# dmlc/difacto

Hardware: AMD Instinct MI355X
Metric: examples/sec (FM SGD worker step, Criteo-shape, V_dim=64) (higher is better)
Workload: dtype f32

## Files before the change

difacto_amd/csrc/dfh_api.hip:

```cpp
#include <algorithm>
#include <chrono>
#include <cstring>
#include <mutex>
#include <new>
#include <thread>

#include <hip/hip_ext.h>
#include <rocprim/rocprim.hpp>

#include "dfh_kernels.hip"
#include "dfh_localize.hip"
#include "dfh_update.hip"
#include "dfh_riders.hip"

using namespace dfh;

namespace dfh {
static thread_local std::string g_err;
void set_error(const std::string& msg) { g_err = msg; }
}

struct dfh_ctx {
  int device = 0;
  hipStream_t stream = nullptr;
// ... 39 lines not shown

namespace {
struct TimeScope {
  dfh_ctx* c;
  int id;
  hipStream_t st;
  hipEvent_t a = nullptr, b = nullptr;
  static hipEvent_t get(dfh_ctx* c) {
    if (!c->pool.empty()) {
      hipEvent_t e = c->pool.back();
      c->pool.pop_back();
      return e;
    }
    hipEvent_t e = nullptr;
    if (hipEventCreate(&e) != hipSuccess) return nullptr;
    return e;
  }
  TimeScope(dfh_ctx* ctx, int kid, hipStream_t s = nullptr) : c(ctx), id(kid), st(s ? s : ctx->stream) {
    if (kid >= DFH_K_COUNT || !((c->timing >> kid) & 1u)) return;
    a = get(c);
    b = get(c);
    if (a && b) (void)hipEventRecord(a, st);
  }
  ~TimeScope() {
    if (!a || !b) return;
    (void)hipEventRecord(b, st);
    c->spans.push_back({id, a, b});
  }
};
}

struct dfh_table {
  dfh_ctx* ctx = nullptr;
  TableView v{};
  uint64_t hslots = 0;
  uint64_t bytes = 0;
  bool has_aux = true;
  bool auto_grow = false;
  uint64_t rows_bound = 0;
  uint64_t grows = 0;
  uint32_t* d_need = nullptr;
  uint32_t* d_rank = nullptr;
  uint32_t* d_urow = nullptr;
  uint32_t* d_total = nullptr;
  size_t aux_cap = 0;
};

struct dfh_batch {
  dfh_ctx* ctx = nullptr;
  size_t max_rows = 0, max_nnz = 0;
  size_t nrows = 0, nnz = 0;
  bool has_value = false;
  bool has_cnt = false;
  bool localized = false;
  uint64_t* d_raw = nullptr;
  uint32_t* d_offset = nullptr;
  float* d_value = nullptr;
  float* d_label = nullptr;
  void* arena = nullptr;
  void* shared_arena = nullptr;
  size_t arena_bytes = 0;
  uint64_t* o_raw = nullptr;
  uint32_t* o_offset = nullptr;
  float* o_value = nullptr;
  float* o_label = nullptr;
  StageLayout stage;
  char* h_stage = nullptr;
  size_t stage_bytes = 0;
  hipEvent_t ev_staged = nullptr;
  bool staged_pending = false;
  double t_prof[6] = {0, 0, 0, 0, 0, 0};
  uint64_t n_prof = 0;
  char* d_stage_view = nullptr;
  bool defer_ready = false;
  uint64_t *d_keys = nullptr, *d_skeys = nullptr;
  uint32_t *d_pos = nullptr, *d_spos = nullptr;
  uint32_t *d_bpos = nullptr;
  uint32_t *d_head = nullptr, *d_uid = nullptr;
  void* d_temp = nullptr;
  size_t temp_bytes = 0;
  uint64_t *d_smp_key = nullptr, *d_spl_key = nullptr, *d_first_key = nullptr, *d_last_key = nullptr;
  uint32_t *d_smp_rank = nullptr, *d_smp_pos = nullptr, *d_spl_pos = nullptr, *d_packed = nullptr, *d_run_off = nullptr,
           *d_bstart = nullptr, *d_btotal = nullptr, *d_nheads = nullptr, *d_lh = nullptr;
  size_t max_tiles = 0;
  int spl_P = 0;
  uint64_t* d_feaids = nullptr;
  float* d_feacnt = nullptr;
  uint32_t *d_col_ptr = nullptr, *d_index = nullptr, *d_s_row = nullptr;
  float* d_s_val = nullptr;
  uint32_t* d_U = nullptr;
  uint2 *d_mid = nullptr, *d_hot = nullptr, *d_few = nullptr;
  SegEnt *d_mid_ent = nullptr, *d_hot_ent = nullptr, *d_few_ent = nullptr;
  SegEnt* d_split_ent = nullptr;
  uint32_t* d_split_ticket = nullptr;
  float* d_split_part = nullptr;
  size_t split_cap = 0;
  int split_sel = 0, split_last = 0;
  bool split_listing = false;
  uint32_t seg_nb = 0;
  uint2* d_uw = nullptr;
  uint32_t *d_urow = nullptr, *d_need = nullptr, *d_rank = nullptr, *d_total = nullptr;
  float *d_pred = nullptr, *d_slope = nullptr, *d_xv = nullptr;
  size_t xv_floats = 0;
  static constexpr size_t kProgDoubles = 2 * PROG_SLOTS + 64;
  double* d_prog = nullptr;
  float nrows_seen = 0;
  hipEvent_t ev_ready = nullptr, ev_free = nullptr;
  bool ready_pending = false, free_pending = false;
  hipStream_t prep = nullptr;
  bool compute_auc = false;
  uint32_t *d_auc_keys = nullptr, *d_auc_skeys = nullptr, *d_auc_lab = nullptr, *d_auc_slab = nullptr;
  uint32_t* d_auc_part = nullptr;
  uint32_t auc_pending_n = 0;
  bool force_radix = false;
  bool force_sort_fallback = false;
  dfh_table* looked_up = nullptr;
  struct GatherSeg { struct dfh_rowbuf* rb; size_t at, n; };
  std::vector<GatherSeg> gsegs;
  GatherSrc gsrc{};
  bool gather_pending = false, gather_fusable = false, gather_any_value = false, loc_fuse_gather = false;
  const uint32_t *g_rows = nullptr, *g_off = nullptr;
  const float* g_lab = nullptr;
  LocView loc_v{};
  EmitOut loc_o{};
  uint32_t loc_gsort = 0;
  bool loc_big = false;
  int pend_stage = RID_STAGES;
};

namespace dfh {
namespace chunks {
inline hipError_t reset_prog(dfh_batch* b, hipStream_t s);
}
}

namespace {
int flush_pending(dfh_batch* b);
void pend_remove(dfh_ctx* c, dfh_batch* b);
inline hipStream_t prep_of(const dfh_batch* b) {
  const dfh_ctx* c = b->ctx;
  return (c->pipeline && b->prep) ? b->prep : c->stream;
}
void phase_begin(dfh_batch* b) {
  dfh_ctx* c = b->ctx;
  if (b->pend_stage < RID_STAGES) (void)flush_pending(b);
  hipStream_t next = c->pipeline ? c->preps[c->next_prep++ % c->nprep] : nullptr;
  if (next && b->prep && next != b->prep && b->ready_pending) {
    (void)hipStreamWaitEvent(next, b->ev_ready, 0);
  }
  b->prep = next;
}
int prep_begin(dfh_batch* b) {
  dfh_ctx* c = b->ctx;
  if (c->pipeline && !b->prep) phase_begin(b);
  if (c->pipeline && b->free_pending) {
    DFH_HIP(hipStreamWaitEvent(prep_of(b), b->ev_free, 0));
    b->free_pending = false;
  }
  return DFH_OK;
}
int prep_end(dfh_batch* b) {
  dfh_ctx* c = b->ctx;
  if (c->pipeline && !b->defer_ready) {
    DFH_HIP(hipEventRecord(b->ev_ready, prep_of(b)));
    b->ready_pending = true;
  }
// ... 1793 lines not shown
  DFH_ARG(c && (out || size_only) && max_rows >= 1 && max_nnz >= 1, "dfh_batch_create: bad argument");
  DFH_ARG(max_nnz < 0xFFFFFFF0ULL && max_rows < 0xFFFFFFF0ULL, "batch too large for 32-bit positions");
  DFH_HIP(hipSetDevice(c->device));
  dfh_batch* b = new (std::nothrow) dfh_batch();
  DFH_ARG(b != nullptr, "out of host memory");
  b->ctx = c;
  b->max_rows = max_rows;
  b->max_nnz = max_nnz;
  const size_t N = max_nnz, B = max_rows;
  size_t sort_bytes = 0, scan_bytes = 0;
  rocprim::radix_sort_pairs(nullptr, sort_bytes, (uint64_t*)nullptr, (uint64_t*)nullptr, (uint32_t*)nullptr,
                            (uint32_t*)nullptr, N, 0, 64, c->stream);
  rocprim::inclusive_scan(nullptr, scan_bytes, (uint32_t*)nullptr, (uint32_t*)nullptr, N, rocprim::plus<uint32_t>(), c->stream);
  size_t auc_bytes = 0;
  rocprim::radix_sort_pairs(nullptr, auc_bytes, (uint32_t*)nullptr, (uint32_t*)nullptr, (uint32_t*)nullptr,
                            (uint32_t*)nullptr, B, 0, 32, c->stream);
  b->temp_bytes = std::max(std::max(sort_bytes, scan_bytes), auc_bytes) + 256;
  char* arena_at = nullptr;
  size_t arena_need = 0;
  bool sizing = true;
#define DFH_ALLOC(ptr, count, type)                                                        \
  do {                                                                                     \
    const size_t bytes__ = (((size_t)(count) * sizeof(type)) + 255) & ~(size_t)255;        \
    if (sizing) {                                                                          \
      arena_need += bytes__;                                                               \
    } else {                                                                               \
      (ptr) = reinterpret_cast<type*>(arena_at);                                           \
      arena_at += bytes__;                                                                 \
    }                                                                                      \
  } while (0)
  for (int pass = 0; pass < 2; ++pass) {
  sizing = pass == 0;
  if (!sizing) {
    if (size_only) {
      *size_only = arena_need;
      delete b;
      return DFH_OK;
    }
    if (shared) {
      b->shared_arena = shared;
      ++shared->refs;
      arena_at = static_cast<char*>(shared->base) + at;
    } else {
      hipError_t e__ = hipMalloc(reinterpret_cast<void**>(&b->arena), arena_need);
      if (e__ != hipSuccess) {
        set_error(std::string("dfh_batch_create: hipMalloc: ") + hipGetErrorString(e__));
        dfh_batch_destroy(b);
        return DFH_ERR_HIP;
      }
      arena_at = static_cast<char*>(b->arena);
    }
  }
  DFH_ALLOC(b->o_raw, N, uint64_t);
  DFH_ALLOC(b->o_offset, B + 1, uint32_t);
  DFH_ALLOC(b->o_value, N, float);
  DFH_ALLOC(b->o_label, B, float);
  b->d_raw = b->o_raw;
  b->d_offset = b->o_offset;
  b->d_value = b->o_value;
  b->d_label = b->o_label;
  DFH_ALLOC(b->d_keys, N, uint64_t);
  DFH_ALLOC(b->d_skeys, N, uint64_t);
  DFH_ALLOC(b->d_pos, N, uint32_t);
  DFH_ALLOC(b->d_spos, N, uint32_t);
  DFH_ALLOC(b->d_bpos, N, uint32_t);
  DFH_ALLOC(b->d_head, N, uint32_t);
  DFH_ALLOC(b->d_uid, N, uint32_t);
  DFH_ALLOC(b->d_temp, b->temp_bytes, char);
  b->max_tiles = (N + LOC_TILE - 1) / LOC_TILE;
  b->stage = StageLayout(max_rows, max_nnz, b->max_tiles);
  DFH_ALLOC(b->d_spl_key, LOC_BIG_BUCKETS, uint64_t);
  DFH_ALLOC(b->d_spl_pos, LOC_BIG_BUCKETS, uint32_t);
  DFH_ALLOC(b->d_smp_key, LOC_BIG_BUCKETS * LOC_OVERSAMPLE, uint64_t);
  DFH_ALLOC(b->d_smp_pos, LOC_BIG_BUCKETS * LOC_OVERSAMPLE, uint32_t);
  DFH_ALLOC(b->d_smp_rank, LOC_BIG_BUCKETS * LOC_OVERSAMPLE, uint32_t);
  DFH_ALLOC(b->d_first_key, LOC_BIG_BUCKETS, uint64_t);
  DFH_ALLOC(b->d_last_key, LOC_BIG_BUCKETS, uint64_t);
  DFH_ALLOC(b->d_packed, N, uint32_t);
  DFH_ALLOC(b->d_run_off, b->max_tiles * LOC_BIG_BUCKETS, uint32_t);
  DFH_ALLOC(b->d_bstart, LOC_BIG_BUCKETS + 1, uint32_t);
  DFH_ALLOC(b->d_btotal, LOC_XCDS * LOC_BIG_BUCKETS, uint32_t);
  DFH_ALLOC(b->d_nheads, LOC_BIG_BUCKETS, uint32_t);
  DFH_ALLOC(b->d_lh, LOC_BIG_BUCKETS, uint32_t);
  DFH_ALLOC(b->d_feaids, N, uint64_t);
  DFH_ALLOC(b->d_feacnt, N, float);
  DFH_ALLOC(b->d_col_ptr, N + 1, uint32_t);
  DFH_ALLOC(b->d_index, N, uint32_t);
  DFH_ALLOC(b->d_s_row, N, uint32_t);
  DFH_ALLOC(b->d_s_val, N, float);
  DFH_ALLOC(b->d_U, 64, uint32_t);
  DFH_ALLOC(b->d_urow, N, uint32_t);
  DFH_ALLOC(b->d_uw, N, uint2);
  DFH_ALLOC(b->d_mid_ent, N / (BWD_SMALL + 1) + 2 * LOC_BIG_BUCKETS + 16, SegEnt);
  DFH_ALLOC(b->d_hot_ent, N / (BWD_MID + 1) + 2 * LOC_BIG_BUCKETS + 16, SegEnt);
  DFH_ALLOC(b->d_few_ent, N / 2 + 2 * LOC_BIG_BUCKETS + 16, SegEnt);
  b->split_cap = 2 * (N / HOT_SPLIT) + 16;
  DFH_ALLOC(b->d_split_ent, b->split_cap, SegEnt);
  DFH_ALLOC(b->d_split_ticket, b->split_cap, uint32_t);
  DFH_ALLOC(b->d_split_part, b->split_cap * UPD_SPLIT_STRIDE, float);
  DFH_ALLOC(b->d_mid, LOC_BIG_BUCKETS, uint2);
  DFH_ALLOC(b->d_hot, LOC_BIG_BUCKETS, uint2);
  DFH_ALLOC(b->d_few, LOC_BIG_BUCKETS, uint2);
  DFH_ALLOC(b->d_need, N, uint32_t);
  DFH_ALLOC(b->d_rank, N, uint32_t);
  DFH_ALLOC(b->d_pred, B, float);
  DFH_ALLOC(b->d_slope, B, float);
  DFH_ALLOC(b->d_prog, dfh_batch::kProgDoubles, double);
  DFH_ALLOC(b->d_auc_keys, B, uint32_t);
  DFH_ALLOC(b->d_auc_skeys, B, uint32_t);
  DFH_ALLOC(b->d_auc_lab, B, uint32_t);
  DFH_ALLOC(b->d_auc_slab, B, uint32_t);
  DFH_ALLOC(b->d_auc_part, AUC_PART_WORDS, uint32_t);
  }
#undef DFH_ALLOC
  b->arena_bytes = arena_need;
  b->d_total = b->d_U + 1;
  const unsigned evf = hipEventDisableTiming | (c->event_flags ? hipEventDisableSystemFence : 0u);
  hipError_t e2 = hipEventCreateWithFlags(&b->ev_ready, evf);
  if (e2 == hipSuccess) e2 = hipEventCreateWithFlags(&b->ev_free, evf);
  if (e2 == hipSuccess) e2 = chunks::reset_prog(b, c->stream);
  if (e2 == hipSuccess) e2 = hipMemsetAsync(b->d_U, 0, 64 * sizeof(uint32_t), c->stream);
  if (e2 == hipSuccess) e2 = hipMemsetAsync(b->d_split_ticket, 0, b->split_cap * sizeof(uint32_t), c->stream);
  if (e2 == hipSuccess) e2 = hipMemsetAsync(b->d_btotal, 0, LOC_XCDS * LOC_BIG_BUCKETS * sizeof(uint32_t), c->stream);
  if (e2 == hipSuccess) e2 = hipMemsetAsync(b->d_urow, 0xFF, N * sizeof(uint32_t), c->stream);
  if (e2 == hipSuccess) e2 = hipMemsetAsync(b->d_uw, 0xFF, N * sizeof(uint2), c->stream);
  if (e2 == hipSuccess && sync) e2 = hipStreamSynchronize(c->stream);
  if (e2 != hipSuccess) {
    set_error(std::string("dfh_batch_create: ") + hipGetErrorString(e2));
    dfh_batch_destroy(b);
    return DFH_ERR_HIP;
  }
  *out = b;
  return DFH_OK;
}

int dfh_batch_create(dfh_ctx* c, size_t max_rows, size_t max_nnz, dfh_batch** out) {
  return batch_create_impl(c, max_rows, max_nnz, out, nullptr, 0, nullptr, true);
}

int dfh_batch_create_many(dfh_ctx* c, int n, size_t max_rows, size_t max_nnz, dfh_batch** out) {
  DFH_ARG(c && out && n >= 1 && n <= 64, "dfh_batch_create_many: 1 <= n <= 64 objects");
  size_t each = 0;
  int rc = batch_create_impl(c, max_rows, max_nnz, nullptr, nullptr, 0, &each, false);
  if (rc) return rc;
  each = (each + 4095) & ~(size_t)4095;
  SharedArena* sa = new (std::nothrow) SharedArena();
  DFH_ARG(sa != nullptr, "out of host memory");
  DFH_HIP(hipSetDevice(c->device));
  if (hipMalloc(&sa->base, each * (size_t)n) != hipSuccess) {
    delete sa;
    set_error("dfh_batch_create_many: hipMalloc failed");
    return DFH_ERR_HIP;
  }
  for (int i = 0; i < n; ++i) out[i] = nullptr;
  sa->refs = 1;
  for (int i = 0; i < n && !rc; ++i) rc = batch_create_impl(c, max_rows, max_nnz, &out[i], sa, each * (size_t)i, nullptr, false);
  if (!rc && hipStreamSynchronize(c->stream) != hipSuccess) {
    set_error("dfh_batch_create_many: hipStreamSynchronize failed");
    rc = DFH_ERR_HIP;
  }
  if (rc) {
    for (int j = 0; j < n; ++j) {
      if (out[j]) dfh_batch_destroy(out[j]);
      out[j] = nullptr;
    }
  }
// ... 36 lines not shown

extern "C" {

int dfh_batch_load_host(dfh_batch* b, size_t nrows, const size_t* offset, const uint64_t* index, const float* value,
                        const float* label) {
  DFH_ARG(b && offset && label, "dfh_batch_load_host: NULL argument");
  DFH_ARG(nrows >= 1 && nrows <= b->max_rows, "dfh_batch_load_host: nrows out of range");
  std::vector<uint32_t> off32;
  int rc = to_u32_offsets(offset, nrows, &off32);
  if (rc) return rc;
  const size_t base = offset[0], nnz = off32[nrows];
  DFH_ARG(nnz <= b->max_nnz, "dfh_batch_load_host: nnz exceeds max_nnz");
  DFH_ARG(nnz == 0 || index, "index is NULL");
  DFH_HIP(hipSetDevice(b->ctx->device));
  rc = phase_own_arrays(b);
  if (rc) return rc;
  hipStream_t s = prep_of(b);
  const StageLayout& L = b->stage;
  rc = ensure_stage(b, L.load_host_bytes, false);
  if (!rc) rc = stage_wait(b);
  if (rc) return rc;
  memcpy(b->h_stage + L.o_off, off32.data(), (nrows + 1) * 4);
  memcpy(b->h_stage + L.o_lab, label, nrows * 4);
  if (nnz) memcpy(b->h_stage + L.o_idx, index + base, nnz * 8);
  if (nnz && value) memcpy(b->h_stage + L.o_val, value + base, nnz * 4);
  DFH_HIP(hipMemcpyAsync(b->d_offset, b->h_stage + L.o_off, (nrows + 1) * 4, hipMemcpyHostToDevice, s));
  DFH_HIP(hipMemcpyAsync(b->d_label, b->h_stage + L.o_lab, nrows * 4, hipMemcpyHostToDevice, s));
  if (nnz) DFH_HIP(hipMemcpyAsync(b->d_raw, b->h_stage + L.o_idx, nnz * 8, hipMemcpyHostToDevice, s));
  if (nnz && value) DFH_HIP(hipMemcpyAsync(b->d_value, b->h_stage + L.o_val, nnz * 4, hipMemcpyHostToDevice, s));
  DFH_HIP(hipEventRecord(b->ev_staged, s));
  b->staged_pending = true;
  batch_loaded(b, nrows, nnz, value != nullptr);
  return DFH_OK;
}

int dfh_batch_load_device(dfh_batch* b, size_t nrows, size_t nnz, const uint32_t* d_offset, const uint64_t* d_index,
                          const float* d_value, const float* d_label) {
  DFH_ARG(b && d_offset && d_label && (nnz == 0 || d_index), "dfh_batch_load_device: NULL argument");
  DFH_ARG(nrows >= 1 && nrows <= b->max_rows && nnz <= b->max_nnz, "dfh_batch_load_device: shape out of range");
  int rc = phase_own_arrays(b);
  if (rc) return rc;
  hipStream_t s = prep_of(b);
  DFH_HIP(hipMemcpyAsync(b->d_offset, d_offset, (nrows + 1) * 4, hipMemcpyDeviceToDevice, s));
  if (nnz) DFH_HIP(hipMemcpyAsync(b->d_raw, d_index, nnz * 8, hipMemcpyDeviceToDevice, s));
  if (nnz && d_value) DFH_HIP(hipMemcpyAsync(b->d_value, d_value, nnz * 4, hipMemcpyDeviceToDevice, s));
  DFH_HIP(hipMemcpyAsync(b->d_label, d_label, nrows * 4, hipMemcpyDeviceToDevice, s));
  batch_loaded(b, nrows, nnz, d_value != nullptr);
  return DFH_OK;
}

int dfh_batch_attach_device(dfh_batch* b, size_t nrows, size_t nnz, const uint32_t* d_offset, const uint64_t* d_index,
                            const float* d_value, const float* d_label) {
  DFH_ARG(b && d_offset && d_label && (nnz == 0 || d_index), "dfh_batch_attach_device: NULL argument");
  DFH_ARG(nrows >= 1 && nrows <= b->max_rows && nnz <= b->max_nnz, "dfh_batch_attach_device: shape out of range");
  phase_begin(b);
  {
    int rc = prep_begin(b);
    if (rc) return rc;
  }
  b->d_offset = const_cast<uint32_t*>(d_offset);
  b->d_raw = const_cast<uint64_t*>(d_index);
  b->d_value = d_value ? const_cast<float*>(d_value) : b->o_value;
  b->d_label = const_cast<float*>(d_label);
  batch_loaded(b, nrows, nnz, d_value != nullptr);
  return DFH_OK;
}

namespace {
void launch_loc_stage(dfh_batch* b, int stage, hipStream_t s, dfh_table* probe = nullptr) {
  const LocView& v = b->loc_v;
  switch (stage) {
    case RID_COUNT:
      if (b->loc_big) hipLaunchKernelGGL(k_loc_count<LOC_BIG_BUCKETS>, dim3(v.ntiles), dim3(LOC_TILE_THREADS), 0, s, v);
      else if (b->loc_fuse_gather) hipLaunchKernelGGL(k_loc_count_gather<LOC_MAX_BUCKETS>, dim3(v.ntiles), dim3(LOC_TILE_THREADS), 0, s, v, b->gsrc);
      else hipLaunchKernelGGL(k_loc_count<LOC_MAX_BUCKETS>, dim3(v.ntiles), dim3(LOC_TILE_THREADS), 0, s, v);
      break;
    case RID_SCATTER:
      if (b->loc_big) hipLaunchKernelGGL(k_loc_scatter<LOC_BIG_BUCKETS>, dim3(v.ntiles), dim3(LOC_TILE_THREADS), 0, s, v);
      else hipLaunchKernelGGL(k_loc_scatter<LOC_MAX_BUCKETS>, dim3(v.ntiles), dim3(LOC_TILE_THREADS), 0, s, v);
      break;
    case RID_SORT:
      hipLaunchKernelGGL(k_loc_sort, dim3(b->loc_gsort), dim3(LOC_SORT_THREADS), loc_sort_smem(), s, v);
      break;
    default:
      if (probe) hipLaunchKernelGGL(k_loc_emit<true>, dim3(b->loc_gsort), dim3(LOC_EMIT_THREADS), 0, s, v, b->loc_o, probe->v, b->d_urow);
      else hipLaunchKernelGGL(k_loc_emit<false>, dim3(b->loc_gsort), dim3(LOC_EMIT_THREADS), 0, s, v, b->loc_o, TableView{}, (uint32_t*)nullptr);
      break;
  }
}

void pend_remove(dfh_ctx* c, dfh_batch* b) {
  auto it = std::find(c->pend.begin(), c->pend.end(), b);
  if (it != c->pend.end()) c->pend.erase(it);
}

int flush_pending(dfh_batch* b) {
  dfh_ctx* c = b->ctx;
  if (b->pend_stage >= RID_STAGES) return DFH_OK;
  {
    TimeScope ts(c, DFH_K_LOCALIZE);
    for (int st = b->pend_stage; st < RID_STAGES; ++st) launch_loc_stage(b, st, c->stream);
  }
  b->pend_stage = RID_STAGES;
  pend_remove(c, b);
  DFH_HIP(hipGetLastError());
  return DFH_OK;
}

void collect_riders(dfh_ctx* c, int slot, bool can_ride, uint32_t main_groups, RiderSet* rs) {
  rs->n = 0;
  rs->ngroups = 0;
  rs->period = 1;
  rs->start = 0;
  rs->first[0] = 0;
  if (!c->single_queue || c->pend.empty()) return;
  for (size_t i = 0; i < c->pend.size(); ++i) {
    dfh_batch* p = c->pend[i];
    while (p->pend_stage < RID_STAGES && c->rider_slot[p->pend_stage] == slot) {
      const int st = p->pend_stage;
      if (c->rider_alone[st] || !can_ride || rs->n == MAX_RIDERS) {
        TimeScope ts(c, DFH_K_LOCALIZE);
        launch_loc_stage(p, st, c->stream);
        ++p->pend_stage;
        continue;
      }
      Rider& r = rs->r[rs->n];
      r.v = p->loc_v;
      r.o = p->loc_o;
      r.kind = (uint32_t)st;
      r.nblk = (st == RID_COUNT || st == RID_SCATTER) ? (uint32_t)p->loc_v.ntiles : p->loc_gsort;
      rs->first[rs->n + 1] = rs->first[rs->n] + ((r.nblk + 7u) & ~7u);
      ++rs->n;
      ++p->pend_stage;
      break;
    }
  }
  for (uint32_t j = 1; j < rs->n; ++j) {
    if (rs->r[j].kind == RID_EMIT && rs->r[0].kind != RID_EMIT) {
      std::swap(rs->r[0], rs->r[j]);
      uint32_t at = 0;
      for (uint32_t q = 0; q < rs->n; ++q) {
        rs->first[q] = at;
        at += (rs->r[q].nblk + 7u) & ~7u;
      }
      rs->first[rs->n] = at;
      break;
    }
  }
  c->pend.erase(std::remove_if(c->pend.begin(), c->pend.end(), [](dfh_batch* p) { return p->pend_stage >= RID_STAGES; }), c->pend.end());
  rs->ngroups = rs->first[rs->n] / 8u;
  for (uint32_t q = rs->n + 1; q <= (uint32_t)MAX_RIDERS; ++q) rs->first[q] = rs->first[rs->n];
  if (rs->ngroups) {
    rs->start = (uint32_t)((uint64_t)main_groups * (uint64_t)c->rider_start[slot] / 100u);
    const uint32_t left = main_groups - rs->start;
    uint32_t per = (uint32_t)std::max(1, c->rider_period[slot]);
    if (rs->ngroups > 1) per = std::min(per, (left + rs->ngroups - 1u) / (rs->ngroups - 1u));
    rs->period = std::max(1u, per);
  }
}

int localize_impl(dfh_batch* b, uint64_t max_index, dfh_table* probe) {
  dfh_ctx* c = b->ctx;
  DFH_HIP(hipSetDevice(c->device));
  const uint32_t N = (uint32_t)b->nnz;
  if (probe && N) {
    if (int rcr = table_reserve(probe, N)) return rcr;
  }
  {
    int rc = prep_begin(b);
    if (rc) return rc;
  }
  hipStream_t s = prep_of(b);
  b->looked_up = nullptr;
  if (b->pend_stage < RID_STAGES) {
    int rc = flush_pending(b);
    if (rc) return rc;
  }
  if (N == 0) {
    if (b->gather_pending) {
      int rcg = gather_alone(b, s);
      if (rcg) return rcg;
    }
    DFH_HIP(hipMemsetAsync(b->d_U, 0, 64 * sizeof(uint32_t), s));
    DFH_HIP(hipMemsetAsync(b->d_col_ptr, 0, 4, s));
    b->seg_nb = 0;
    b->localized = true;
    return prep_end(b);
  }
  const int g = grid_for_threads(N, c);
  TimeScope* tsp = new TimeScope(c, DFH_K_LOCALIZE, s);
  int P = 0;
  bool cold = true;
  if (b->spl_P > 0 && N / (uint32_t)b->spl_P >= (uint32_t)LOC_MIN_AVG && N / (uint32_t)b->spl_P <= (uint32_t)LOC_MAX_AVG) {
    P = b->spl_P;
    cold = false;
  } else {
#ifndef DFH_LOC_SMALL_AVG
#define DFH_LOC_SMALL_AVG 192
#endif
    const size_t avg_bucket = N <= 65536u ? (size_t)DFH_LOC_SMALL_AVG : (size_t)LOC_AVG_BUCKET;
    const size_t P_want = (N + avg_bucket - 1) / avg_bucket;
    if (P_want <= (size_t)LOC_MAX_BUCKETS) P = (int)std::max<size_t>(1, P_want);
    else if (N / LOC_MAX_BUCKETS <= (uint32_t)LOC_MAX_AVG) P = LOC_MAX_BUCKETS;
    else if (P_want <= (size_t)LOC_BIG_BUCKETS) P = (int)P_want;
    else if (N / LOC_BIG_BUCKETS <= (uint32_t)LOC_MAX_AVG) P = LOC_BIG_BUCKETS;
  }
  b->loc_fuse_gather = b->gather_pending && b->gather_fusable && !cold && P > 0 && P <= LOC_MAX_BUCKETS && !b->force_radix &&
                       !c->single_queue && !getenv("DFH_GATHER_ALONE");
  if (b->gather_pending && !b->loc_fuse_gather) {
    int rcg = gather_alone(b, s);
    if (rcg) return rcg;
  }
  if (P > 0 && !b->force_radix) {
    LocView& v = b->loc_v;
    v.raw = b->d_raw;
    v.n = N;
    v.max_index = max_index;
    v.P = P;
    const bool big = P > LOC_MAX_BUCKETS;
    v.bstride = big ? LOC_BIG_BUCKETS : LOC_MAX_BUCKETS;
    v.ntiles = (int)((N + LOC_TILE - 1) / LOC_TILE);
    v.force_global = b->force_sort_fallback ? 1 : 0;
    v.tb = N > 1 ? std::min(16, __builtin_clz(N - 1)) : 16;
    v.nrows = (uint32_t)b->nrows;
    v.offset = b->d_offset;
    v.rowid = b->d_pos;
    v.smp_key = b->d_smp_key;
    v.smp_pos = b->d_smp_pos;
    v.smp_rank = b->d_smp_rank;
    v.spl_key = b->d_spl_key;
    v.spl_pos = b->d_spl_pos;
    v.packed = b->d_packed;
    v.run_off = b->d_run_off;
    v.btotal = b->d_btotal;
    v.bstart = b->d_bstart;
    v.bkeys = b->d_keys;
    v.bpos = b->d_bpos;
    v.skeys = b->d_skeys;
    v.spos = b->d_spos;
    v.first_key = b->d_first_key;
    v.last_key = b->d_last_key;
    v.nheads = b->d_nheads;
    v.lh = b->d_lh;
    EmitOut& o = b->loc_o;
    o.value = b->has_value ? b->d_value : (const float*)nullptr;
    o.feaids = b->d_feaids;
    o.col_ptr = b->d_col_ptr;
    o.index = b->d_index;
    o.s_row = b->d_s_row;
    o.s_val = b->d_s_val;
    o.d_U = b->d_U;
    o.sl.mid = b->d_mid;
    o.sl.mid_ent = b->d_mid_ent;
    o.sl.hot = b->d_hot;
    o.sl.hot_ent = b->d_hot_ent;
    o.sl.few = b->d_few;
    o.sl.few_ent = b->d_few_ent;
    v.split_n = b->d_U + 2;
    b->loc_big = big;
#ifndef DFH_LOC_GRID_CAP
#define DFH_LOC_GRID_CAP 1024
#endif
    b->loc_gsort = (unsigned)std::min<int>(P, big ? LOC_BIG_BUCKETS : DFH_LOC_GRID_CAP);
    if (cold && P > 1) {
      const uint32_t S = (uint32_t)P * LOC_OVERSAMPLE;
      const uint32_t nt = (S + 255) / 256;
      hipLaunchKernelGGL(k_ss_sample, dim3(nt), dim3(256), 0, s, v);
      hipLaunchKernelGGL(k_ss_rank, dim3(nt * nt), dim3(256), 0, s, v);
      hipLaunchKernelGGL(k_loc_splitters, dim3(nt), dim3(256), 0, s, v);
    }
    if (c->single_queue && !cold && !big && !probe) {
      b->pend_stage = 0;
      c->pend.push_back(b);
    } else {
      for (int st = 0; st < RID_STAGES; ++st) {
        launch_loc_stage(b, st, s, probe);
        if (st == RID_COUNT && b->loc_fuse_gather) {
          int rcg = gather_queued(b, s);
          b->loc_fuse_gather = false;
          if (rcg) return rcg;
        }
      }
    }
    b->spl_P = P;
    b->seg_nb = (uint32_t)P;
  } else {
    hipLaunchKernelGGL(k_rdx_keys, dim3(g), dim3(256), 0, s, b->d_raw, N, max_index, b->d_keys, b->d_pos);
    size_t tb = b->temp_bytes;
    DFH_HIP(rocprim::radix_sort_pairs(b->d_temp, tb, b->d_keys, b->d_skeys, b->d_pos, b->d_spos, (size_t)N, 0, 64, s));
    hipLaunchKernelGGL(k_rdx_heads, dim3(g), dim3(256), 0, s, b->d_skeys, N, b->d_head);
    tb = b->temp_bytes;
    DFH_HIP(rocprim::inclusive_scan(b->d_temp, tb, b->d_head, b->d_uid, (size_t)N, rocprim::plus<uint32_t>(), s));
    hipLaunchKernelGGL(k_rdx_emit, dim3(g), dim3(256), 0, s, b->d_skeys, b->d_spos, b->d_head, b->d_uid, N, (uint32_t)b->nrows,
                       b->d_offset, b->has_value ? b->d_value : (const float*)nullptr, b->d_feaids, b->d_col_ptr, b->d_index,
                       b->d_s_row, b->d_s_val, b->d_U);
    hipLaunchKernelGGL(k_seg_lists_reset, dim3(1), dim3(64), 0, s, b->d_mid, b->d_hot, b->d_few, b->d_U + 2);
    hipLaunchKernelGGL(k_seg_lists, dim3((unsigned)std::max<size_t>(1, std::min<size_t>((N + 1023) / 1024, 256))), dim3(1024), 0, s,
                       b->d_col_ptr, b->d_U, b->d_mid, b->d_hot, b->d_few, b->d_mid_ent, b->d_hot_ent, b->d_few_ent);
    b->seg_nb = 1;
    if (probe)
      hipLaunchKernelGGL(k_lookup, dim3(grid_for_threads(b->nnz, c)), dim3(256), 0, s, probe->v, b->d_feaids, b->d_U, 0u, b->d_urow,
                         (const float*)nullptr, b->d_col_ptr, 0, (uint32_t*)nullptr, 0, (uint2*)nullptr, AucFin{nullptr, 0u, nullptr});
  }
  delete tsp;
  DFH_HIP(hipGetLastError());
  b->localized = true;
  b->has_cnt = false;
  if (probe) b->looked_up = probe;
  return prep_end(b);
}
}


int dfh_localize(dfh_batch* b, uint64_t max_index) {
  DFH_ARG(b && b->nrows > 0, "dfh_localize: no batch loaded");
  DFH_ARG(max_index != 0, "max_index must be nonzero");
  return localize_impl(b, max_index, nullptr);
}

int dfh_localize_lookup(dfh_table* t, dfh_batch* b, uint64_t max_index) {
  DFH_ARG(t && b && t->ctx == b->ctx, "dfh_localize_lookup: bad argument");
  DFH_ARG(b->nrows > 0, "dfh_localize_lookup: no batch loaded");
  DFH_ARG(max_index != 0, "max_index must be nonzero");
  return localize_impl(b, max_index, t);
}

// ... 384 lines not shown
```

difacto_amd/csrc/dfh_localize.hip:

```cpp
#ifndef DFH_LOCALIZE_HIP_
#define DFH_LOCALIZE_HIP_
#include "dfh_internal.h"
#include "dfh_feed_layout.h"

namespace dfh {

constexpr int LOC_OVERSAMPLE = 8;
constexpr int LOC_MAX_BUCKETS = 1024;
constexpr int LOC_BIG_BUCKETS = 4096;
constexpr int LOC_AVG_BUCKET = 384;
constexpr int LOC_MIN_AVG = 48;
constexpr int LOC_MAX_AVG = 700;
constexpr int LOC_LDS_CAP = 1024;
#ifndef DFH_LOC_TILE_THREADS
#define DFH_LOC_TILE_THREADS 1024
#endif
constexpr int LOC_TILE_THREADS = DFH_LOC_TILE_THREADS;
constexpr int LOC_PER_THREAD = LOC_TILE / LOC_TILE_THREADS;
constexpr int LOC_SORT_THREADS = 256;
constexpr int LOC_EMIT_THREADS = 256;

struct LocView {
  const uint64_t* raw;
  uint32_t n;
  uint64_t max_index;
  int P;
  int bstride;
  int ntiles;
  int force_global;
  int tb;
  uint32_t nrows;
  const uint32_t* offset;
  const uint32_t* rowid;
  uint64_t* smp_key;
  uint32_t* smp_pos;
  uint32_t* smp_rank;
  uint64_t* spl_key;
  uint32_t* spl_pos;
  uint32_t* packed;
  uint32_t* run_off;
  uint32_t* btotal;
  uint32_t* bstart;
  uint64_t* bkeys;
  uint32_t* bpos;
  uint64_t* skeys;
  uint32_t* spos;
  uint64_t* first_key;
  uint64_t* last_key;
  uint32_t* nheads;
  uint32_t* lh;
  uint32_t* split_n;
};

struct SegListsOut {
  uint2* mid;
  SegEnt* mid_ent;
  uint2* hot;
  SegEnt* hot_ent;
  uint2* few;
  SegEnt* few_ent;
};

__device__ __forceinline__ uint64_t make_key(uint64_t id, uint64_t max_index) {
  const uint64_t m = (max_index == ~0ULL) ? (id == ~0ULL ? 0ULL : id) : id % max_index;
  return reverse_bytes(m);
}

constexpr int LOC_XCDS = 8;

__device__ __forceinline__ bool comp_less(uint64_t ka, uint32_t pa, uint64_t kb, uint32_t pb) {
  return ka < kb || (ka == kb && pa < pb);
}

template <bool MAX>
__device__ __forceinline__ uint32_t wave_inclusive(uint32_t x) {
#define DFH_DPP_STEP(ctrl, row_mask)                                                                      \
  {                                                                                                       \
    const uint32_t y = (uint32_t)__builtin_amdgcn_update_dpp(0, (int)x, ctrl, row_mask, 0xf, false);    \
    x = MAX ? max(x, y) : x + y;                                                                          \
  }
  DFH_DPP_STEP(0x111, 0xf)
  DFH_DPP_STEP(0x112, 0xf)
  DFH_DPP_STEP(0x114, 0xf)
  DFH_DPP_STEP(0x118, 0xf)
  DFH_DPP_STEP(0x142, 0xa)
  DFH_DPP_STEP(0x143, 0xc)
#undef DFH_DPP_STEP
  return x;
}

template <bool MAX, int NWAVES>
__device__ __forceinline__ uint32_t block_exclusive(uint32_t val, uint32_t* wtot , uint32_t* total) {
  static_assert(NWAVES <= 64, "one lane per wave");
  const int lane = (int)(threadIdx.x & 63);
  const int w = __builtin_amdgcn_readfirstlane((int)(threadIdx.x >> 6));
  const uint32_t s = wave_inclusive<MAX>(val);
  __syncthreads();
  if (lane == 63) wtot[w] = s;
  __syncthreads();
  const uint32_t x = wave_inclusive<MAX>(lane < NWAVES ? wtot[lane] : 0u);
  const uint32_t before = w ? (uint32_t)__builtin_amdgcn_readlane((int)x, w - 1) : 0u;
  if (total) *total = (uint32_t)__builtin_amdgcn_readlane((int)x, NWAVES - 1);
  const uint32_t prev = (uint32_t)__builtin_amdgcn_update_dpp(0, (int)s, 0x138, 0xf, 0xf, false);
  return MAX ? max(before, prev) : before + prev;
}
template <int NWAVES>
__device__ __forceinline__ uint32_t block_exclusive_scan(uint32_t val, uint32_t* wsum , uint32_t* total) {
  return block_exclusive<false, NWAVES>(val, wsum, total);
}
template <int NWAVES>
__device__ __forceinline__ uint32_t block_exclusive_max(uint32_t val, uint32_t* wmax , uint32_t* total) {
  return block_exclusive<true, NWAVES>(val, wmax, total);
}

__device__ __forceinline__ uint32_t ss_sample_pos(uint32_t t, uint32_t stride, uint32_t n) {
  const uint32_t j = (uint32_t)(splitmix64(t) >> 33) % stride;
  return min(t * stride + j, n - 1);
}

__global__ void __launch_bounds__(256) k_ss_sample(LocView v) {
  const uint32_t S = (uint32_t)v.P * LOC_OVERSAMPLE;
  const uint32_t stride = max(1u, v.n / S);
  for (uint32_t t = blockIdx.x * blockDim.x + threadIdx.x; t < S; t += gridDim.x * blockDim.x) {
    const uint32_t i = ss_sample_pos(t, stride, v.n);
    v.smp_key[t] = make_key(v.raw[i], v.max_index);
    v.smp_pos[t] = i << v.tb;
    v.smp_rank[t] = 0;
  }
}

__global__ void __launch_bounds__(256) k_ss_rank(LocView v) {
  __shared__ uint64_t ck[256];
  __shared__ uint32_t cp[256];
// ... 448 lines not shown
struct BucketSummary {
  uint32_t nheads, lh;
  uint64_t first_key, last_key;
};
template <bool WRITE>
__device__ __forceinline__ BucketSummary loc_bucket_summary(const uint64_t* sk, const uint32_t* sp, uint32_t n, uint64_t* ok,
                                                            uint32_t* op, uint32_t (*red)[LOC_SORT_THREADS / 64]) {
  uint32_t cnt = 0, last = 0;
  uint32_t t0 = threadIdx.x;
  asm volatile("" : "+v"(t0));
  for (uint32_t t = t0; t < n; t += LOC_SORT_THREADS) {
    const uint64_t k = sk[t];
    if (WRITE) {
      ok[t] = k;
      op[t] = sp[t];
    }
    if (t + 1 < n && sk[t + 1] != k) {
      ++cnt;
      last = t + 1;
    }
  }
  cnt = (uint32_t)__builtin_amdgcn_readlane((int)wave_inclusive<false>(cnt), 63);
  last = (uint32_t)__builtin_amdgcn_readlane((int)wave_inclusive<true>(last), 63);
  if ((threadIdx.x & 63) == 0) {
    red[0][threadIdx.x >> 6] = cnt;
    red[1][threadIdx.x >> 6] = last;
  }
  __syncthreads();
  BucketSummary r;
  r.nheads = 1;
  r.lh = 0;
  r.first_key = 0;
  r.last_key = 0;
  if (threadIdx.x == 0) {
    for (int w = 0; w < LOC_SORT_THREADS / 64; ++w) {
      r.nheads += red[0][w];
      r.lh = max(r.lh, red[1][w]);
    }
    r.first_key = sk[0];
    r.last_key = sk[n - 1];
  }
  return r;
}

__device__ __forceinline__ void loc_sort_block(const LocView& v, const uint32_t bid, const uint32_t nblk, char* smem) {
  uint64_t* ak = reinterpret_cast<uint64_t*>(smem);
  uint64_t* bk = ak + LOC_LDS_CAP;
  uint32_t* ap = reinterpret_cast<uint32_t*>(bk + LOC_LDS_CAP);
  uint32_t* bp = ap + LOC_LDS_CAP;
  uint32_t (*red)[LOC_SORT_THREADS / 64] = reinterpret_cast<uint32_t (*)[LOC_SORT_THREADS / 64]>(bp + LOC_LDS_CAP);
  for (uint32_t b = bid; b < (uint32_t)v.P; b += nblk) {
    __syncthreads();
    const uint32_t beg = v.bstart[b], end = v.bstart[b + 1];
    const uint32_t n = end - beg;
    if (threadIdx.x < LOC_XCDS) v.btotal[threadIdx.x * v.bstride + b] = 0;
    if (n == 0) {
      if (threadIdx.x == 0) {
        v.nheads[b] = 0;
        v.lh[b] = 0;
        v.first_key[b] = 0;
        v.last_key[b] = 0;
      }
      continue;
    }
    BucketSummary sm;
    if (n <= LOC_LDS_CAP && !v.force_global) {
      const bool in_a = loc_sort_bucket_lds(v, beg, n, ak, ap, bk, bp);
      sm = loc_bucket_summary<true>(in_a ? ak : bk, in_a ? ap : bp, n, v.skeys + beg, v.spos + beg, red);
    } else {
      loc_sort_bucket_global(v, beg, n);
      sm = loc_bucket_summary<false>(v.skeys + beg, v.spos + beg, n, nullptr, nullptr, red);
    }
    if (threadIdx.x == 0) {
      v.nheads[b] = sm.nheads;
      v.lh[b] = sm.lh;
      v.first_key[b] = sm.first_key;
      v.last_key[b] = sm.last_key;
    }
  }
}
__global__ void __launch_bounds__(LOC_SORT_THREADS) k_loc_sort(LocView v) {
  extern __shared__ __attribute__((aligned(16))) char smem[];
  loc_sort_block(v, blockIdx.x, gridDim.x, smem);
}

template <int NW, bool PROBE>
__device__ __forceinline__ void loc_emit_bucket(const LocView& v, uint32_t b, uint32_t beg, uint32_t n, const uint64_t* sk,
                                                const uint32_t* sp, uint32_t cont, uint32_t ubase, uint32_t carry1,
                                                const float* __restrict__ value,
                                                uint64_t* __restrict__ feaids, uint32_t* __restrict__ col_ptr,
                                                uint32_t* __restrict__ index, uint32_t* __restrict__ s_row,
                                                float* __restrict__ s_val, uint32_t* __restrict__ d_U, const SegListsOut& sl,
                                                uint32_t* wsum, uint32_t* wmax, uint32_t* n_mid, uint32_t* n_hot,
                                                uint32_t* n_few, const TableView& tab, uint32_t* __restrict__ urow) {
  const uint32_t P = (uint32_t)v.P;
  const uint32_t moff = beg / (BWD_SMALL + 1) + 2 * b, hoff = beg / (BWD_MID + 1) + 2 * b, foff = beg / 2 + 2 * b;
  uint32_t run_heads = 0, run_max1 = carry1;
  for (uint32_t base = 0; base < n; base += blockDim.x) {
    const uint32_t t = base + threadIdx.x;
    const uint32_t i = beg + t;
    const bool valid = t < n;
    uint64_t key = 0;
    uint32_t tag = 0;
    bool head = false;
    if (valid) {
      key = sk[t];
      tag = sp[t];
      head = t == 0 ? !cont : key != sk[t - 1];
    }
    const uint32_t pos = tag >> v.tb;
    uint32_t nh, mx;
    const uint32_t ex = block_exclusive_scan<NW>(head ? 1u : 0u, wsum, &nh);
    const uint32_t pm = block_exclusive_max<NW>(head ? i + 1 : 0u, wmax, &mx);
    if (valid) {
      const uint32_t incl = run_heads + ex + (head ? 1u : 0u);
      const uint32_t uid = ubase + incl - 1;
      const uint32_t prev1 = max(run_max1, pm);
      if (head) {
        feaids[uid] = key;
        col_ptr[uid] = i;
        if (PROBE) urow[uid] = find_or_insert(tab, key);
        if (prev1) {
          const uint32_t len = i - (prev1 - 1);
          const SegEnt e = make_uint4(uid - 1, prev1 - 1, i, 0u);
          if (len > BWD_MID) sl.hot_ent[hoff + atomicAdd(n_hot, 1u)] = e;
          else if (len > BWD_SMALL) sl.mid_ent[moff + atomicAdd(n_mid, 1u)] = e;
          else if (len > 1) sl.few_ent[foff + atomicAdd(n_few, 1u)] = e;
        }
      }
      index[pos] = uid;
      uint32_t row = tag & ((1u << v.tb) - 1u);
      {
        const uint32_t step = 1u << v.tb;
        uint32_t lo = 0, hi = v.nrows > row ? (v.nrows - 1u - row) >> v.tb : 0u;
        while (lo < hi) {
          const uint32_t mid = (lo + hi + 1u) >> 1;
          if (v.offset[row + mid * step] <= pos) lo = mid; else hi = mid - 1u;
        }
        row += lo * step;
      }
      s_row[i] = row;
      if (value) s_val[i] = value[pos];
      if (i == v.n - 1) {
        *d_U = uid + 1;
        col_ptr[uid + 1] = v.n;
        const uint32_t lbeg = head ? i : prev1 - 1, len = v.n - lbeg;
        const SegEnt e = make_uint4(uid, lbeg, v.n, 0u);
        if (len > BWD_MID) sl.hot_ent[hoff + atomicAdd(n_hot, 1u)] = e;
        else if (len > BWD_SMALL) sl.mid_ent[moff + atomicAdd(n_mid, 1u)] = e;
        else if (len > 1) sl.few_ent[foff + atomicAdd(n_few, 1u)] = e;
      }
    }
    run_heads += nh;
    run_max1 = max(run_max1, mx);
  }
  if (P > 1) {
    const uint64_t N = v.n;
    const uint64_t m0 = max((uint64_t)beg * P / N + ((uint64_t)beg * P % N ? 1u : 0u), (uint64_t)1);
    const uint64_t e1 = (uint64_t)(beg + n) * P;
    const uint64_t m1 = min(e1 / N + (e1 % N ? 1u : 0u), (uint64_t)P);
    for (uint64_t m = m0 + threadIdx.x; m < m1; m += blockDim.x) {
      const uint32_t i = (uint32_t)(m * N / P);
      if ((i * (uint64_t)P + N - 1) / N == m) {
        v.spl_key[m - 1] = sk[i - beg];
        v.spl_pos[m - 1] = sp[i - beg];
      }
    }
  }
  __syncthreads();
  if (threadIdx.x == 0) {
    sl.mid[b] = make_uint2(*n_mid, moff);
    sl.hot[b] = make_uint2(*n_hot, hoff);
    sl.few[b] = make_uint2(*n_few, foff);
  }
}

struct EmitOut {
  const float* value;
  uint64_t* feaids;
  uint32_t* col_ptr;
  uint32_t* index;
  uint32_t* s_row;
  float* s_val;
  uint32_t* d_U;
  SegListsOut sl;
};

template <bool PROBE>
__device__ __forceinline__ void loc_emit_block(const LocView& v, const EmitOut& o, const TableView& tab, uint32_t* __restrict__ urow,
                                               const uint32_t bid, const uint32_t nblk, char* smem) {
  constexpr int NW = LOC_EMIT_THREADS / 64;
  uint32_t* wsum = reinterpret_cast<uint32_t*>(smem);
  uint32_t* wmax = wsum + NW;
  uint32_t& sh_cont = wmax[NW];
  uint32_t& n_mid = wmax[NW + 1];
  uint32_t& n_hot = wmax[NW + 2];
  uint32_t& n_few = wmax[NW + 3];
  const SegListsOut& sl = o.sl;
  const uint32_t P = (uint32_t)v.P;
  for (uint32_t b = bid; b < P; b += nblk) {
    __syncthreads();
    const uint32_t beg = v.bstart[b], end = v.bstart[b + 1];
    const uint32_t n = end - beg;
    if (threadIdx.x == 0) {
      n_mid = 0;
      n_hot = 0;
      n_few = 0;
      if (n == 0) {
        sl.mid[b] = make_uint2(0u, 0u);
        sl.hot[b] = make_uint2(0u, 0u);
        sl.few[b] = make_uint2(0u, 0u);
      }
    }
    if (n == 0) continue;
    uint32_t part = 0, carry1 = 0;
    for (uint32_t q0 = threadIdx.x; q0 <= b; q0 += LOC_EMIT_THREADS) {
      const uint32_t bq = v.bstart[q0], nq = v.bstart[q0 + 1] - bq;
      if (nq == 0) continue;
      int p = (int)q0 - 1;
      while (p >= 0 && v.bstart[p + 1] == v.bstart[p]) --p;
      const uint32_t c = (p >= 0 && v.first_key[q0] == v.last_key[p]) ? 1u : 0u;
      if (q0 == b) {
        sh_cont = c;
      } else {
        part += v.nheads[q0] - c;
        const uint32_t l = v.lh[q0];
        if (l > 0) carry1 = max(carry1, bq + l + 1);
        else if (!c) carry1 = max(carry1, bq + 1);
      }
    }
    uint32_t ubase, carry_all;
    block_exclusive_scan<NW>(part, wsum, &ubase);
    block_exclusive_max<NW>(carry1, wmax, &carry_all);
    __syncthreads();
    loc_emit_bucket<NW, PROBE>(v, b, beg, n, v.skeys + beg, v.spos + beg, sh_cont, ubase, carry_all, o.value, o.feaids, o.col_ptr,
                               o.index, o.s_row, o.s_val, o.d_U, sl, wsum, wmax, &n_mid, &n_hot, &n_few, tab, urow);
  }
}

template <bool PROBE>
__global__ void __launch_bounds__(LOC_EMIT_THREADS) k_loc_emit(LocView v, EmitOut o, TableView tab, uint32_t* __restrict__ urow) {
  __shared__ __attribute__((aligned(16))) char smem[loc_emit_smem()];
  loc_emit_block<PROBE>(v, o, tab, urow, blockIdx.x, gridDim.x, smem);
}

}
#endif
```

Baseline: 87.89 million.

## Precompute per-bucket stitch prefix data in a single-block kernel before emit

Adds a one-block stitch kernel that computes, once per batch, each bucket's unique-id base, carry max and continuation flag using block-wide scans over all buckets. The emit kernel then reads these from a small array instead of having every bucket's block rescan all preceding buckets, which was quadratic in the bucket count and walked backward over empty buckets. The cost is one extra kernel launch and a serial single-block pass, and it applies only to the non-big localize path.

```diff
diff --git a/difacto_amd/csrc/dfh_api.hip b/difacto_amd/csrc/dfh_api.hip
--- a/difacto_amd/csrc/dfh_api.hip
+++ b/difacto_amd/csrc/dfh_api.hip
@@ -145,6 +145,7 @@
   uint64_t *d_smp_key = nullptr, *d_spl_key = nullptr, *d_first_key = nullptr, *d_last_key = nullptr;
   uint32_t *d_smp_rank = nullptr, *d_smp_pos = nullptr, *d_spl_pos = nullptr, *d_packed = nullptr, *d_run_off = nullptr,
            *d_bstart = nullptr, *d_btotal = nullptr, *d_nheads = nullptr, *d_lh = nullptr;
+  uint4* d_stitch = nullptr;
   size_t max_tiles = 0;
   int spl_P = 0;
   uint64_t* d_feaids = nullptr;
@@ -2104,6 +2105,7 @@
   DFH_ALLOC(b->d_btotal, LOC_XCDS * LOC_BIG_BUCKETS, uint32_t);
   DFH_ALLOC(b->d_nheads, LOC_BIG_BUCKETS, uint32_t);
   DFH_ALLOC(b->d_lh, LOC_BIG_BUCKETS, uint32_t);
+  DFH_ALLOC(b->d_stitch, LOC_BIG_BUCKETS, uint4);
   DFH_ALLOC(b->d_feaids, N, uint64_t);
   DFH_ALLOC(b->d_feacnt, N, float);
   DFH_ALLOC(b->d_col_ptr, N + 1, uint32_t);
@@ -2306,10 +2308,16 @@
     case RID_SORT:
       hipLaunchKernelGGL(k_loc_sort, dim3(b->loc_gsort), dim3(LOC_SORT_THREADS), loc_sort_smem(), s, v);
       break;
-    default:
-      if (probe) hipLaunchKernelGGL(k_loc_emit<true>, dim3(b->loc_gsort), dim3(LOC_EMIT_THREADS), 0, s, v, b->loc_o, probe->v, b->d_urow);
-      else hipLaunchKernelGGL(k_loc_emit<false>, dim3(b->loc_gsort), dim3(LOC_EMIT_THREADS), 0, s, v, b->loc_o, TableView{}, (uint32_t*)nullptr);
+    default: {
+      LocView ve = v;
+      if (!b->loc_big) {
+        ve.stitch = b->d_stitch;
+        hipLaunchKernelGGL(k_loc_stitch, dim3(1), dim3(LOC_STITCH_THREADS), 0, s, ve);
+      }
+      if (probe) hipLaunchKernelGGL(k_loc_emit<true>, dim3(b->loc_gsort), dim3(LOC_EMIT_THREADS), 0, s, ve, b->loc_o, probe->v, b->d_urow);
+      else hipLaunchKernelGGL(k_loc_emit<false>, dim3(b->loc_gsort), dim3(LOC_EMIT_THREADS), 0, s, ve, b->loc_o, TableView{}, (uint32_t*)nullptr);
       break;
+    }
   }
 }
 
@@ -2466,6 +2474,7 @@
     v.last_key = b->d_last_key;
     v.nheads = b->d_nheads;
     v.lh = b->d_lh;
+    v.stitch = nullptr;
     EmitOut& o = b->loc_o;
     o.value = b->has_value ? b->d_value : (const float*)nullptr;
     o.feaids = b->d_feaids;
diff --git a/difacto_amd/csrc/dfh_localize.hip b/difacto_amd/csrc/dfh_localize.hip
--- a/difacto_amd/csrc/dfh_localize.hip
+++ b/difacto_amd/csrc/dfh_localize.hip
@@ -49,6 +49,7 @@
   uint64_t* last_key;
   uint32_t* nheads;
   uint32_t* lh;
+  uint4* stitch;
   uint32_t* split_n;
 };
 
@@ -663,6 +664,66 @@
 __global__ void __launch_bounds__(LOC_SORT_THREADS) k_loc_sort(LocView v) {
   extern __shared__ __attribute__((aligned(16))) char smem[];
   loc_sort_block(v, blockIdx.x, gridDim.x, smem);
+}
+
+constexpr int LOC_STITCH_THREADS = 256;
+constexpr int LOC_STITCH_ROUNDS = LOC_MAX_BUCKETS / LOC_STITCH_THREADS;
+__global__ void __launch_bounds__(LOC_STITCH_THREADS) k_loc_stitch(LocView v) {
+  constexpr int NW = LOC_STITCH_THREADS / 64;
+  __shared__ uint64_t lk[LOC_MAX_BUCKETS];
+  __shared__ uint32_t wtot[NW];
+  const uint32_t P = (uint32_t)v.P;
+  uint64_t fk[LOC_STITCH_ROUNDS];
+  uint32_t nh[LOC_STITCH_ROUNDS];
+  uint32_t hd[LOC_STITCH_ROUNDS];
+  {
+    auto kmid = [](const uint64_t* a) {
+      uint32_t o = 2 * LOC_STITCH_THREADS + threadIdx.x;
+      asm volatile("" : "+v"(o));
+      return a + o;
+    };
+    uint64_t lq[LOC_STITCH_ROUNDS];
+    uint32_t bq[LOC_STITCH_ROUNDS], l[LOC_STITCH_ROUNDS];
+    static_assert(LOC_STITCH_ROUNDS == 4, "the asm statements name four rounds");
+#pragma unroll
+    for (int r = 0; r < LOC_STITCH_ROUNDS; ++r) lq[r] = kmid(v.last_key)[(r - 2) * LOC_STITCH_THREADS];
+#pragma unroll
+    for (int r = 0; r < LOC_STITCH_ROUNDS; ++r) {
+      const uint32_t q = (uint32_t)r * LOC_STITCH_THREADS + threadIdx.x;
+      nh[r] = v.nheads[q];
+      bq[r] = v.bstart[q];
+      l[r] = v.lh[q];
+    }
+    asm volatile("" : "+v"(lq[0]), "+v"(lq[1]), "+v"(lq[2]), "+v"(lq[3]) : : "memory");
+#pragma unroll
+    for (int r = 0; r < LOC_STITCH_ROUNDS; ++r) lk[r * LOC_STITCH_THREADS + threadIdx.x] = lq[r];
+#pragma unroll
+    for (int r = 0; r < LOC_STITCH_ROUNDS; ++r) fk[r] = kmid(v.first_key)[(r - 2) * LOC_STITCH_THREADS];
+    asm volatile("" : "+v"(nh[0]), "+v"(nh[1]), "+v"(nh[2]), "+v"(nh[3]), "+v"(bq[0]), "+v"(bq[1]), "+v"(bq[2]), "+v"(bq[3]),
+                      "+v"(l[0]), "+v"(l[1]), "+v"(l[2]), "+v"(l[3]));
+#pragma unroll
+    for (int r = 0; r < LOC_STITCH_ROUNDS; ++r) {
+      const uint32_t q = (uint32_t)r * LOC_STITCH_THREADS + threadIdx.x;
+      nh[r] = q < P ? nh[r] : 0u;
+      hd[r] = nh[r] ? (l[r] ? ((bq[r] + l[r] + 1u) << 1) | 1u : (bq[r] + 1u) << 1) : 0u;
+    }
+  }
+  uint32_t run_p = 0, run_u = 0, run_c = 0;
+#pragma unroll
+  for (int r = 0; r < LOC_STITCH_ROUNDS; ++r) {
+    if ((uint32_t)r * LOC_STITCH_THREADS >= P) break;
+    const uint32_t q = (uint32_t)r * LOC_STITCH_THREADS + threadIdx.x;
+    uint32_t tot_p, tot_u, tot_c;
+    const uint32_t p1 = max(run_p, block_exclusive_max<NW>(nh[r] ? q + 1u : 0u, wtot, &tot_p));
+    const uint32_t c = (nh[r] && p1 && fk[r] == lk[p1 - 1u]) ? 1u : 0u;
+    const uint32_t c1 = (hd[r] & 1u) || !c ? hd[r] >> 1 : 0u;
+    const uint32_t ub = run_u + block_exclusive_scan<NW>(nh[r] - c, wtot, &tot_u);
+    const uint32_t ca = max(run_c, block_exclusive_max<NW>(c1, wtot, &tot_c));
+    if (q < P) v.stitch[q] = make_uint4(ub, ca, c, 0u);
+    run_p = max(run_p, tot_p);
+    run_u += tot_u;
+    run_c = max(run_c, tot_c);
+  }
 }
 
 template <int NW, bool PROBE>
@@ -794,27 +855,35 @@
       }
     }
     if (n == 0) continue;
-    uint32_t part = 0, carry1 = 0;
-    for (uint32_t q0 = threadIdx.x; q0 <= b; q0 += LOC_EMIT_THREADS) {
-      const uint32_t bq = v.bstart[q0], nq = v.bstart[q0 + 1] - bq;
-      if (nq == 0) continue;
-      int p = (int)q0 - 1;
-      while (p >= 0 && v.bstart[p + 1] == v.bstart[p]) --p;
-      const uint32_t c = (p >= 0 && v.first_key[q0] == v.last_key[p]) ? 1u : 0u;
-      if (q0 == b) {
-        sh_cont = c;
-      } else {
-        part += v.nheads[q0] - c;
-        const uint32_t l = v.lh[q0];
-        if (l > 0) carry1 = max(carry1, bq + l + 1);
-        else if (!c) carry1 = max(carry1, bq + 1);
-      }
-    }
-    uint32_t ubase, carry_all;
-    block_exclusive_scan<NW>(part, wsum, &ubase);
-    block_exclusive_max<NW>(carry1, wmax, &carry_all);
-    __syncthreads();
-    loc_emit_bucket<NW, PROBE>(v, b, beg, n, v.skeys + beg, v.spos + beg, sh_cont, ubase, carry_all, o.value, o.feaids, o.col_ptr,
+    uint32_t cont, ubase, carry_all;
+    if (v.stitch) {
+      const uint4 st = v.stitch[b];
+      ubase = st.x;
+      carry_all = st.y;
+      cont = st.z;
+    } else {
+      uint32_t part = 0, carry1 = 0;
+      for (uint32_t q0 = threadIdx.x; q0 <= b; q0 += LOC_EMIT_THREADS) {
+        const uint32_t bq = v.bstart[q0], nq = v.bstart[q0 + 1] - bq;
+        if (nq == 0) continue;
+        int p = (int)q0 - 1;
+        while (p >= 0 && v.bstart[p + 1] == v.bstart[p]) --p;
+        const uint32_t c = (p >= 0 && v.first_key[q0] == v.last_key[p]) ? 1u : 0u;
+        if (q0 == b) {
+          sh_cont = c;
+        } else {
+          part += v.nheads[q0] - c;
+          const uint32_t l = v.lh[q0];
+          if (l > 0) carry1 = max(carry1, bq + l + 1);
+          else if (!c) carry1 = max(carry1, bq + 1);
+        }
+      }
+      block_exclusive_scan<NW>(part, wsum, &ubase);
+      block_exclusive_max<NW>(carry1, wmax, &carry_all);
+      __syncthreads();
+      cont = sh_cont;
+    }
+    loc_emit_bucket<NW, PROBE>(v, b, beg, n, v.skeys + beg, v.spos + beg, cont, ubase, carry_all, o.value, o.feaids, o.col_ptr,
                                o.index, o.s_row, o.s_val, o.d_U, sl, wsum, wmax, &n_mid, &n_hot, &n_few, tab, urow);
   }
 }
```

New measurement: 88.62 million (median of 5 runs). About the same (+0.8%).
